# arkworks-rs/circom-compat

Hardware: NVIDIA H100
Metric: groth16_proofs_per_sec_bn254_2p20 (higher is better)
Workload: dtype u32x8 (254-bit Montgomery integers)

## Files before the change

### circom_compat_b200/csrc/msm.cu

```cuda
#include <algorithm>
#include <type_traits>
#include <vector>
#include "msm.cuh"
#include "util.cuh"

namespace b2g {

std::atomic<uint64_t> g_launch_count{0};

template <class C, class F>
__global__ void __launch_bounds__(128) msm_table_kernel(const void* __restrict__ bases, uint32_t n, int c, int nwin, void* __restrict__ table) {
    uint32_t i = blockIdx.x * blockDim.x + threadIdx.x;
    if (i >= n) return;
    using Pt = typename C::Pt; using Aff = typename C::Aff; using E = typename F::elem;
    Aff p = aff_load<F>(bases, i);
    if (C::aff_is_inf(p)) {
        Aff z; z.x = F::zero(); z.y = F::zero();
        for (int w = 0; w < nwin; w++) aff_store<F>(table, (size_t)w * n + i, z);
        return;
    }
    Pt pts[MSM_MAX_WIN];
    E pre[MSM_MAX_WIN];
    Pt cur = C::from_affine(p);
    E acc = F::one();
    for (int w = 0; w < nwin; w++) {
        pts[w] = cur;
        pre[w] = acc;
        acc = F::mul(acc, cur.zzz);
        if (w + 1 < nwin) for (int j = 0; j < c; j++) cur = C::dbl(cur);
    }
    E inv = F::inv(acc);
    for (int w = nwin - 1; w >= 0; w--) {
        E iz = F::mul(inv, pre[w]);
        inv = F::mul(inv, pts[w].zzz);
        Aff a;
        a.y = F::mul(pts[w].y, iz);
        a.x = F::mul(pts[w].x, F::mul(F::sqr(pts[w].zz), F::sqr(iz)));
        aff_store<F>(table, (size_t)w * n + i, a);
    }
}

template <class C, class F>
__global__ void __launch_bounds__(256) msm_validate_kernel(const void* __restrict__ bases, uint32_t n, uint32_t* __restrict__ bad) {
    uint32_t i = blockIdx.x * blockDim.x + threadIdx.x;
    if (i >= n) return;
    if (!aff_on_curve<C, F>(aff_load<F>(bases, i))) atomicMax(bad, i + 1u);
}

__global__ void __launch_bounds__(256) msm_canon_kernel(const fe* __restrict__ scalars, uint32_t n, uint32_t scalar_stride, int scalars_mont, fe* __restrict__ canon_out) {
    uint32_t i = blockIdx.x * blockDim.x + threadIdx.x;
    if (i >= n) return;
    scalars += (size_t)blockIdx.y * scalar_stride;
    canon_out += (size_t)blockIdx.y * n;
    fe k = fe_load_nc(&scalars[i]);
    if (scalars_mont) k = Fr::to_canonical(k);
    fe_store(&canon_out[i], k);
}

__device__ __forceinline__ uint32_t msm_window_bits(const uint32_t* __restrict__ k, int c, int w) {
    const uint32_t off = (uint32_t)w * (uint32_t)c, limb = off >> 5, sh = off & 31u;
    if (limb >= 8) return 0u;
    uint64_t v = __ldg(&k[limb]);
    if (limb + 1 < 8 && sh + (uint32_t)c > 32u) v |= (uint64_t)__ldg(&k[limb + 1]) << 32;
    return (uint32_t)(v >> sh) & ((1u << c) - 1u);
}

__device__ __forceinline__ int32_t msm_digit_at(const uint32_t* __restrict__ k, int c, int w) {
    const uint32_t half = 1u << (c - 1);
    uint32_t carry = 0;
    for (int v = w - 1; v >= 0; v--) {
        const uint32_t b = msm_window_bits(k, c, v);
        if (b >= half) { carry = 1; break; }
        if (b < half - 1) break;
    }
    const uint32_t coef = msm_window_bits(k, c, w) + carry;
    const uint32_t cout = (coef + half) >> c;
    return (int32_t)coef - (int32_t)(cout << c);
}

constexpr int MSM_LEADER_ROUNDS = 2;

__global__ void __launch_bounds__(256) msm_count_kernel(const fe* __restrict__ canon, uint32_t n, int c, int nwin, uint32_t nb, uint32_t* __restrict__ counts) {
    canon += (size_t)blockIdx.y * n;
    counts += (size_t)blockIdx.y * nb;
    const uint64_t tid = (uint64_t)blockIdx.x * blockDim.x + threadIdx.x;
    const uint32_t w = (uint32_t)(tid / n), i = (uint32_t)(tid % n);
    int32_t d = 0;
    if (w < (uint32_t)nwin) d = msm_digit_at(canon[i].l, c, (int)w);
    const uint32_t b = d ? (uint32_t)(d < 0 ? -d : d) - 1u : 0xffffffffu;
    const uint32_t lane = threadIdx.x & 31;
    bool pending = d != 0;
    {
        const uint32_t hot = __ballot_sync(0xffffffffu, pending && b == 0u);
        if (hot) {
            if ((int)lane == __ffs(hot) - 1) atomicAdd(&counts[0], (uint32_t)__popc(hot));
            if (b == 0u) pending = false;
        }
    }
    #pragma unroll
    for (int round = 0; round < MSM_LEADER_ROUNDS; round++) {
        const uint32_t pend = __ballot_sync(0xffffffffu, pending);
        if (!pend) break;
        const int leader = __ffs(pend) - 1;
        const uint32_t lb = __shfl_sync(0xffffffffu, b, leader);
        const bool mine = pending && b == lb;
        const uint32_t same = __ballot_sync(0xffffffffu, mine);
        if ((int)lane == leader) atomicAdd(&counts[lb], (uint32_t)__popc(same));
        if (mine) pending = false;
    }
    if (pending) atomicAdd(&counts[b], 1u);
}

__global__ void __launch_bounds__(1024) msm_scan_kernel(const uint32_t* __restrict__ counts, uint32_t nb, uint32_t* __restrict__ offsets,
                                                        uint32_t* __restrict__ cursor) {
    __shared__ uint32_t warp_sums[32];
    __shared__ uint32_t carry_s;
    const uint32_t tid = threadIdx.x, per = (nb + 1023u) / 1024u;
    const uint32_t lo = tid * per, hi = min(lo + per, nb);
    uint32_t s = 0;
    if ((per & 3u) == 0 && hi == lo + per) {
        const uint4* v4 = reinterpret_cast<const uint4*>(counts + lo);
        #pragma unroll 4
        for (uint32_t j = 0; j < per / 4; j++) { const uint4 q = __ldg(&v4[j]); s += q.x + q.y + q.z + q.w; }
    } else {
        for (uint32_t j = lo; j < hi; j++) s += counts[j];
    }
    uint32_t v = s;
    #pragma unroll
    for (int d = 1; d < 32; d <<= 1) { uint32_t t = __shfl_up_sync(0xffffffffu, v, d); if ((tid & 31) >= (uint32_t)d) v += t; }
    if ((tid & 31) == 31) warp_sums[tid >> 5] = v;
    __syncthreads();
    if (tid < 32) {
        uint32_t w = warp_sums[tid], x = w;
        #pragma unroll
        for (int d = 1; d < 32; d <<= 1) { uint32_t t = __shfl_up_sync(0xffffffffu, x, d); if (tid >= (uint32_t)d) x += t; }
        warp_sums[tid] = x - w;
        if (tid == 31) carry_s = x;
    }
    __syncthreads();
    uint32_t run = warp_sums[tid >> 5] + v - s;
    for (uint32_t j = lo; j < hi; j++) { offsets[j] = run; cursor[j] = 0; run += counts[j]; }
    if (tid == 0) offsets[nb] = carry_s;
}

__global__ void __launch_bounds__(256) msm_scatter_kernel(const fe* __restrict__ canon, uint32_t n, uint32_t row_stride, int c, int nwin, uint32_t nb,
                                   const uint32_t* __restrict__ offsets, uint32_t* __restrict__ cursor, uint32_t* __restrict__ entries) {
    canon += (size_t)blockIdx.y * n;
    offsets += (size_t)blockIdx.y * nb;
    cursor += (size_t)blockIdx.y * nb;
    const uint64_t tid = (uint64_t)blockIdx.x * blockDim.x + threadIdx.x;
    const uint32_t w = (uint32_t)(tid / n), i = (uint32_t)(tid % n);
    int32_t d = 0;
    if (w < (uint32_t)nwin) d = msm_digit_at(canon[i].l, c, (int)w);
    const uint32_t b = d ? (uint32_t)(d < 0 ? -d : d) - 1u : 0xffffffffu;
    const uint32_t lane = threadIdx.x & 31;
    const uint32_t entry = (w * row_stride + i) | (d < 0 ? 0x80000000u : 0u);
    bool pending = d != 0;
    {
        const uint32_t hot = __ballot_sync(0xffffffffu, pending && b == 0u);
        if (hot) {
            const int leader = __ffs(hot) - 1;
            uint32_t base = 0;
            if ((int)lane == leader) base = atomicAdd(&cursor[0], (uint32_t)__popc(hot));
            base = __shfl_sync(0xffffffffu, base, leader);
            if (pending && b == 0u) {
                entries[offsets[0] + base + (uint32_t)__popc(hot & ((1u << lane) - 1u))] = entry;
                pending = false;
            }
        }
    }
    #pragma unroll
    for (int round = 0; round < MSM_LEADER_ROUNDS; round++) {
        const uint32_t pend = __ballot_sync(0xffffffffu, pending);
        if (!pend) break;
        const int leader = __ffs(pend) - 1;
        const uint32_t lb = __shfl_sync(0xffffffffu, b, leader);
        const bool mine = pending && b == lb;
        const uint32_t same = __ballot_sync(0xffffffffu, mine);
        uint32_t base = 0;
        if ((int)lane == leader) base = atomicAdd(&cursor[lb], (uint32_t)__popc(same));
        base = __shfl_sync(0xffffffffu, base, leader);
        if (mine) {
            entries[offsets[b] + base + (uint32_t)__popc(same & ((1u << lane) - 1u))] = entry;
            pending = false;
        }
    }
    if (pending) entries[offsets[b] + atomicAdd(&cursor[b], 1u)] = entry;
}

__global__ void __launch_bounds__(1024) msm_aff_levels_kernel(uint32_t nb, int rounds, uint32_t* const* __restrict__ off) {
    __shared__ uint32_t warp_sums[32];
    __shared__ uint32_t carry_s;
    const uint32_t tid = threadIdx.x, per = (nb + 1023u) / 1024u;
    const uint32_t lo = min(tid * per, nb), hi = min(lo + per, nb);
    for (int k = 1; k <= rounds; k++) {
        const uint32_t* prev = off[k - 1];
        uint32_t* cur = off[k];
        uint32_t s = 0;
        for (uint32_t j = lo; j < hi; j++) s += (prev[j + 1] - prev[j] + 1u) >> 1;
        uint32_t v = s;
        #pragma unroll
        for (int d = 1; d < 32; d <<= 1) { uint32_t t = __shfl_up_sync(0xffffffffu, v, d); if ((tid & 31) >= (uint32_t)d) v += t; }
        if ((tid & 31) == 31) warp_sums[tid >> 5] = v;
        __syncthreads();
        if (tid < 32) {
            uint32_t w = warp_sums[tid], x = w;
            #pragma unroll
            for (int d = 1; d < 32; d <<= 1) { uint32_t t = __shfl_up_sync(0xffffffffu, x, d); if (tid >= (uint32_t)d) x += t; }
            warp_sums[tid] = x - w;
            if (tid == 31) carry_s = x;
        }
        __syncthreads();
        uint32_t run = warp_sums[tid >> 5] + v - s;
        for (uint32_t j = lo; j < hi; j++) { cur[j] = run; run += (prev[j + 1] - prev[j] + 1u) >> 1; }
        if (tid == 0) cur[nb] = carry_s;
        __syncthreads();
    }
}

__global__ void __launch_bounds__(256) msm_aff_src_kernel(const uint32_t* __restrict__ off_prev, const uint32_t* __restrict__ off_cur, uint32_t nb,
                                                          uint32_t* __restrict__ src) {
    const uint32_t total = off_cur[nb];
    for (uint32_t q = blockIdx.x * blockDim.x + threadIdx.x; q < total; q += gridDim.x * blockDim.x) {
        uint32_t lo = 0, hi = nb;
        while (hi - lo > 1) { const uint32_t mid = (lo + hi) >> 1; if (off_cur[mid] <= q) lo = mid; else hi = mid; }
        const uint32_t j = q - off_cur[lo];
        const uint32_t p0 = off_prev[lo], cnt = off_prev[lo + 1] - p0;
        src[q] = (p0 + 2u * j) | ((2u * j + 1u < cnt) ? 0x80000000u : 0u);
    }
}

enum : int { AFF_COPY_P = 0, AFF_COPY_Q = 1, AFF_INF = 2, AFF_ADD = 3, AFF_DBL = 4 };

template <class C, class F, bool LEVEL0>
__device__ __forceinline__ int aff_fetch(const void* __restrict__ table, const uint32_t* __restrict__ entries, const void* __restrict__ prev,
                                         uint32_t s, typename C::Aff& P, typename C::Aff& Q, typename F::elem& d) {
    const uint32_t i0 = s & 0x7fffffffu;
    const bool pair = (s >> 31) != 0;
    if (LEVEL0) {
        const uint32_t e0 = entries[i0];
        P = aff_load<F>(table, (size_t)(e0 & 0x7fffffffu));
        if (e0 >> 31) P.y = F::neg(P.y);
        if (pair) {
            const uint32_t e1 = entries[i0 + 1];
            Q = aff_load<F>(table, (size_t)(e1 & 0x7fffffffu));
            if (e1 >> 31) Q.y = F::neg(Q.y);
        }
    } else {
        P = aff_load<F>(prev, (size_t)i0);
        if (pair) Q = aff_load<F>(prev, (size_t)i0 + 1);
    }
    if (!pair) return AFF_COPY_P;
    if (C::aff_is_inf(P)) return AFF_COPY_Q;
    if (C::aff_is_inf(Q)) return AFF_COPY_P;
    if (F::eq(P.x, Q.x)) {
        if (F::eq(P.y, Q.y) && !F::is_zero(P.y)) { d = F::dbl(P.y); return AFF_DBL; }
        return AFF_INF;
    }
    d = F::sub(Q.x, P.x);
    return AFF_ADD;
}

template <class C, class F, bool LEVEL0>
__global__ void __launch_bounds__(128) msm_aff_prod_kernel(const void* __restrict__ table, const uint32_t* __restrict__ entries, const void* __restrict__ prev,
                                                           const uint32_t* __restrict__ src, const uint32_t* __restrict__ off_cur, uint32_t nb,
                                                           void* __restrict__ pref, void* __restrict__ totals) {
    using E = typename F::elem; using Aff = typename C::Aff;
    const uint32_t total = off_cur[nb];
    const uint32_t t = blockIdx.x * blockDim.x + threadIdx.x, stride = gridDim.x * blockDim.x;
    E run = F::one();
// ... 298 lines not shown
            for (int i = top; i >= 0; i--) { m = C::dbl(m); if ((base >> i) & 1u) C::add(m, run); }
            C::add(acc, m);
        }
    }
    Pt r = block_sum_points<C, F, TailThreads<F>::N>(acc, sh);
    if (threadIdx.x == 0) pt_store<F>(partials, blockIdx.x, r);
}

template <class C, class F>
__global__ void __launch_bounds__(TailThreads<F>::N) msm_sum_kernel(const void* __restrict__ pts, uint32_t count, void* __restrict__ out, size_t out_stride) {
    using Pt = typename C::Pt;
    extern __shared__ __align__(32) unsigned char smem_raw[];
    Pt* sh = reinterpret_cast<Pt*>(smem_raw);
    pts = (const char*)pts + (size_t)blockIdx.x * count * sizeof(Pt);
    out = (char*)out + (size_t)blockIdx.x * out_stride;
    Pt acc = C::infinity();
    for (uint32_t i = threadIdx.x; i < count; i += TailThreads<F>::N) { Pt q = pt_load<F>(pts, i); C::add(acc, q); }
    Pt r = block_sum_points<C, F, TailThreads<F>::N>(acc, sh);
    if (threadIdx.x == 0) pt_store<F>(out, 0, r);
}

static uint32_t env_u32(const char* name, uint32_t dflt) {
    const char* v = getenv(name);
    if (!v || !*v) return dflt;
    long x = strtol(v, nullptr, 10);
    return x > 0 ? (uint32_t)x : dflt;
}

void msm_validate_points(const void* pts_dev, uint32_t n, bool g2, cudaStream_t st, const char* what) {
    if (n == 0) return;
    struct Flag { uint32_t* d = nullptr; ~Flag() { if (d) cudaFree(d); } } flag;
    uint32_t bad = 0;
    CUDA_CHECK(cudaMalloc(&flag.d, 4));
    CUDA_CHECK(cudaMemsetAsync(flag.d, 0, 4, st));
    if (g2) msm_validate_kernel<G2, Fq2><<<(n + 255) / 256, 256, 0, st>>>(pts_dev, n, flag.d);
    else msm_validate_kernel<G1, Fq><<<(n + 255) / 256, 256, 0, st>>>(pts_dev, n, flag.d);
    g_launch_count += 1;
    CUDA_CHECK(cudaMemcpyAsync(&bad, flag.d, 4, cudaMemcpyDeviceToHost, st));
    CUDA_CHECK(cudaStreamSynchronize(st));
    if (bad) throw_error(B2G_E_INPUT, std::string(g2 ? "G2" : "G1") + " point " + std::to_string(bad - 1) + " of " + what + " is not on the curve");
}

template <class C, class F>
static void msm_build_table_t(MsmPlan& plan, const void* bases_dev, uint32_t n, cudaStream_t st) {
    const size_t aff = 2 * Bytes<F>::ELEM;
    uint32_t c = env_u32("B2G_MSM_C", (uint32_t)msm_pick_c(n ? n : 1));
    if (c < 8 || c > 22) throw_error(B2G_E_SHAPE, "B2G_MSM_C must be in [8, 22]");
    plan.n = n; plan.c = (int)c; plan.nwin = msm_nwin(plan.c); plan.nbuckets = 1u << (plan.c - 1);
    if (n == 0) { plan.table = nullptr; return; }
    if ((uint64_t)n * plan.nwin >= (1ull << 31)) throw_error(B2G_E_SHAPE, "msm: n * windows exceeds 2^31 table rows");
    msm_validate_points(bases_dev, n, plan.g2, st, "the query slice");
    CUDA_CHECK(cudaMalloc(&plan.table, (size_t)n * plan.nwin * aff));
    msm_table_kernel<C, F><<<(n + 127) / 128, 128, 0, st>>>(bases_dev, n, plan.c, plan.nwin, plan.table);
    g_launch_count += 1;
    CUDA_CHECK(cudaGetLastError());
}

void msm_build_table(MsmPlan& plan, const void* bases_dev, uint32_t n, bool g2, cudaStream_t st) {
    plan.g2 = g2;
    if (g2) msm_build_table_t<G2, Fq2>(plan, bases_dev, n, st);
    else msm_build_table_t<G1, Fq>(plan, bases_dev, n, st);
}

void msm_free_table(MsmPlan& plan) { if (plan.table) cudaFree(plan.table); plan.table = nullptr; }

void msm_scratch_alloc(MsmScratch& s, uint32_t n, int nwin, uint32_t nbuckets_one, bool g2, bool with_sort, uint32_t count) {
    s.g2 = g2; s.cap_n = n; s.cap_nwin = nwin; s.cap_buckets = nbuckets_one; s.cap_count = count;
    s.chunk = env_u32(g2 ? "B2G_MSM_CHUNK_G2" : "B2G_MSM_CHUNK", env_u32("B2G_MSM_CHUNK", 64));
    const size_t pt = (g2 ? 4 * 64 : 4 * 32);
    const size_t nent = (size_t)n * nwin * count;
    const size_t nbuckets = (size_t)nbuckets_one * count;
    const size_t nchunks = (nent + s.chunk - 1) / s.chunk + 1;
    s.reduce_chunk = env_u32("B2G_MSM_REDUCE_CHUNK", MSM_REDUCE_CHUNK_DEFAULT);
    {
        const char* bulk_env = getenv("B2G_ACC_BULK");
        s.bulk = bulk_env && *bulk_env ? *bulk_env == '1' : !g2;
    }
    const size_t npart = ((size_t)nbuckets_one / (s.reduce_chunk * 32) + 64) * count;
    if (with_sort) {
        CUDA_CHECK(cudaMalloc(&s.counts, (size_t)nbuckets * 4));
        CUDA_CHECK(cudaMalloc(&s.offsets, ((size_t)nbuckets + 1) * 4));
        CUDA_CHECK(cudaMalloc(&s.cursor, (size_t)nbuckets * 4));
        CUDA_CHECK(cudaMalloc(&s.entries, (nent + 8) * 4));
        CUDA_CHECK(cudaMalloc(&s.scalars_canon, ((size_t)n * count + 1) * sizeof(fe)));
    }
    CUDA_CHECK(cudaMalloc(&s.big_list, (size_t)nbuckets * 4));
    CUDA_CHECK(cudaMalloc(&s.big_count, 4));
    CUDA_CHECK(cudaMalloc(&s.frag_first, nchunks * pt));
    CUDA_CHECK(cudaMalloc(&s.frag_last, nchunks * pt));
    CUDA_CHECK(cudaMalloc(&s.buckets, (size_t)nbuckets * pt));
    CUDA_CHECK(cudaMalloc(&s.partials, (npart + 1) * pt));
    CUDA_CHECK(cudaMalloc(&s.result, pt)); s.result_owned = true;
    {
        int rounds = 0;
        const char* ov = getenv("B2G_MSM_AFFINE_ROUNDS");
        if (ov && *ov) { long x = strtol(ov, nullptr, 10); rounds = x < 0 ? 0 : (x > MSM_AFF_MAX_ROUNDS ? MSM_AFF_MAX_ROUNDS : (int)x); }
        s.aff_cap_rounds = rounds;
        s.aff_nmax[0] = (uint32_t)nent;
        for (int k = 1; k <= rounds; k++) s.aff_nmax[k] = s.aff_nmax[k - 1] / 2 + (uint32_t)(nbuckets / 2) + 1;
        if (rounds) {
            const size_t elem = g2 ? 64 : 32, aff = 2 * elem;
            if (with_sort) {
                std::vector<uint32_t*> offs(MSM_AFF_MAX_ROUNDS + 1, nullptr);
                offs[0] = s.offsets;
                for (int k = 1; k <= rounds; k++) {
                    CUDA_CHECK(cudaMalloc(&s.aff_off[k], ((size_t)nbuckets + 1) * 4));
                    CUDA_CHECK(cudaMalloc(&s.aff_src[k], ((size_t)s.aff_nmax[k] + 1) * 4));
                    offs[k] = s.aff_off[k];
                }
                s.aff_off[0] = s.offsets;
                CUDA_CHECK(cudaMalloc(&s.aff_off_dev, (MSM_AFF_MAX_ROUNDS + 1) * sizeof(uint32_t*)));
                CUDA_CHECK(cudaMemcpy(s.aff_off_dev, offs.data(), (MSM_AFF_MAX_ROUNDS + 1) * sizeof(uint32_t*), cudaMemcpyHostToDevice));
            }
            CUDA_CHECK(cudaMalloc(&s.aff_list[0], ((size_t)s.aff_nmax[1] + 1) * aff));
            if (rounds > 1) CUDA_CHECK(cudaMalloc(&s.aff_list[1], ((size_t)s.aff_nmax[2] + 1) * aff));
            const size_t threads1 = ((size_t)s.aff_nmax[1] + MSM_AFF_M - 1) / MSM_AFF_M + 128;
            CUDA_CHECK(cudaMalloc(&s.aff_pref, ((size_t)s.aff_nmax[1] + 1) * elem));
            CUDA_CHECK(cudaMalloc(&s.aff_totals, threads1 * elem));
            CUDA_CHECK(cudaMalloc(&s.aff_tscratch, threads1 * elem));
        }
    }
    if (env_u32("B2G_MSM_TAIL_PRIORITY", 1) == 1) {
        int least = 0, greatest = 0;
        CUDA_CHECK(cudaDeviceGetStreamPriorityRange(&least, &greatest));
        CUDA_CHECK(cudaStreamCreateWithPriority(&s.tail, cudaStreamNonBlocking, greatest));
        CUDA_CHECK(cudaEventCreateWithFlags(&s.ev_acc, cudaEventDisableTiming));
        CUDA_CHECK(cudaEventCreateWithFlags(&s.ev_tail, cudaEventDisableTiming));
    }
}

void msm_scratch_free(MsmScratch& s) {
    void* ptrs[] = {s.counts, s.offsets, s.cursor, s.entries, s.big_list, s.big_count, s.frag_first, s.frag_last,
                    s.buckets, s.partials, s.result_owned ? s.result : nullptr, s.scalars_canon,
                    s.aff_list[0], s.aff_list[1], s.aff_pref, s.aff_totals, s.aff_tscratch, s.aff_off_dev};
    for (void* p : ptrs) if (p) cudaFree(p);
    for (int k = 1; k <= MSM_AFF_MAX_ROUNDS; k++) { if (s.aff_off[k]) cudaFree(s.aff_off[k]); if (s.aff_src[k]) cudaFree(s.aff_src[k]); }
    if (s.tail) { cudaStreamDestroy(s.tail); cudaEventDestroy(s.ev_acc); cudaEventDestroy(s.ev_tail); }
    s = MsmScratch();
}

void msm_sort(const MsmPlan& plan, MsmScratch& s, const fe* scalars_dev, uint32_t n, bool scalars_mont, cudaStream_t st, uint32_t count,
              uint32_t scalar_stride) {
    if (n > plan.n) n = plan.n;
    s.sorted_n = n; s.sorted_count = count;
    if (n == 0 || plan.table == nullptr) return;
    if (n > s.cap_n || plan.nwin > s.cap_nwin || plan.nbuckets > s.cap_buckets || count > s.cap_count || !s.entries) throw_error(B2G_E_SHAPE, "msm: sort scratch too small");
    const uint32_t nb = plan.nbuckets * count;
    constexpr unsigned SORT_CTA = 256;
    CUDA_CHECK(cudaMemsetAsync(s.counts, 0, (size_t)nb * 4, st));
    const dim3 pair_grid((unsigned)(((uint64_t)n * plan.nwin + SORT_CTA - 1) / SORT_CTA), count);
    msm_canon_kernel<<<dim3((n + SORT_CTA - 1) / SORT_CTA, count), SORT_CTA, 0, st>>>(scalars_dev, n, scalar_stride ? scalar_stride : n, scalars_mont ? 1 : 0, s.scalars_canon);
    msm_count_kernel<<<pair_grid, SORT_CTA, 0, st>>>(s.scalars_canon, n, plan.c, plan.nwin, plan.nbuckets, s.counts);
    msm_scan_kernel<<<1, 1024, 0, st>>>(s.counts, nb, s.offsets, s.cursor);
    msm_scatter_kernel<<<pair_grid, SORT_CTA, 0, st>>>(s.scalars_canon, n, plan.n, plan.c, plan.nwin, plan.nbuckets, s.offsets, s.cursor, s.entries);
    g_launch_count += 4;
    s.aff_rounds = s.aff_off_dev ? s.aff_cap_rounds : 0;
    if (s.aff_rounds) {
        msm_aff_levels_kernel<<<1, 1024, 0, st>>>(nb, s.aff_rounds, s.aff_off_dev);
        for (int k = 1; k <= s.aff_rounds; k++) {
            const unsigned blocks = (unsigned)std::min<uint64_t>(((uint64_t)s.aff_nmax[k] + 255) / 256, 1u << 20);
            msm_aff_src_kernel<<<blocks, 256, 0, st>>>(s.aff_off[k - 1], s.aff_off[k], nb, s.aff_src[k]);
        }
        g_launch_count += 1 + s.aff_rounds;
    }
    CUDA_CHECK(cudaGetLastError());
}

template <class C, class F>
static void launch_accumulate(const void* table, const uint32_t* entries, const uint32_t* offsets, uint32_t nb, uint32_t chunk, uint32_t nruns,
                              const MsmScratch& s, bool bulk, cudaStream_t st) {
    constexpr bool g2 = std::is_same<F, Fq2>::value;
    constexpr uint32_t runs_per_cta = g2 ? 64u : 128u;
    const uint32_t slab_words = bulk && (size_t)chunk * runs_per_cta * 4 <= MSM_SLAB_MAX_BYTES ? chunk * runs_per_cta : 0u;
    const unsigned blocks = (unsigned)(((uint64_t)nruns + runs_per_cta - 1) / runs_per_cta);
    if constexpr (g2)
        msm_accumulate_g2_kernel<<<blocks, 128, (size_t)slab_words * 4, st>>>(table, entries, offsets, nb, chunk, s.buckets, s.frag_first, s.frag_last, slab_words);
    else
        msm_accumulate_kernel<C, F><<<blocks, 128, (size_t)slab_words * 4, st>>>(table, entries, offsets, nb, chunk, s.buckets, s.frag_first, s.frag_last, slab_words);
}

template <class C, class F>
static void msm_accumulate_t(const MsmPlan& plan, const MsmScratch& sorted, MsmScratch& s, cudaStream_t st) {
    using Pt = typename C::Pt;
    const size_t ptb = sizeof(Pt);
    const uint32_t n = sorted.sorted_n, count = sorted.sorted_count;
    const size_t rstride = s.result_stride ? s.result_stride : ptb;
    if (n == 0 || plan.table == nullptr) { CUDA_CHECK(cudaMemset2DAsync(s.result, rstride, 0, ptb, count, st)); return; }
    if (plan.nbuckets > s.cap_buckets || n > s.cap_n || plan.nwin > s.cap_nwin || count > s.cap_count) throw_error(B2G_E_SHAPE, "msm: accumulate scratch too small");
    const uint32_t nb = plan.nbuckets * count, chunk = s.chunk;
    CUDA_CHECK(cudaMemsetAsync(s.big_count, 0, 4, st));
    const uint64_t nent = (uint64_t)n * plan.nwin * count;
    const uint32_t nthreads = (uint32_t)((nent + chunk - 1) / chunk);
    if (s.prof0) CUDA_CHECK(cudaEventRecord(s.prof0, st));
    int rounds = sorted.aff_rounds < s.aff_cap_rounds ? sorted.aff_rounds : s.aff_cap_rounds;
    if (rounds && (sorted.aff_nmax[1] > s.aff_nmax[1] || !s.aff_list[0])) rounds = 0;
    const uint32_t* offsets = sorted.offsets;
    if (rounds) {
        const void* prev = nullptr;
        for (int k = 1; k <= rounds; k++) {
            const uint32_t nk = sorted.aff_nmax[k];
            const unsigned blocks = (unsigned)(((uint64_t)nk + (uint64_t)MSM_AFF_M * 128 - 1) / ((uint64_t)MSM_AFF_M * 128));
            const uint32_t stride = blocks * 128u, U = (stride + MSM_AFF_S - 1) / MSM_AFF_S;
            void* out = s.aff_list[(k - 1) & 1];
            if (k == 1) {
                msm_aff_prod_kernel<C, F, true><<<blocks, 128, 0, st>>>(plan.table, sorted.entries, nullptr, sorted.aff_src[k], sorted.aff_off[k], nb, s.aff_pref, s.aff_totals);
                msm_aff_invert_kernel<F><<<(U + 63) / 64, 64, 0, st>>>(s.aff_totals, s.aff_tscratch, stride, U);
                msm_aff_apply_kernel<C, F, true><<<blocks, 128, 0, st>>>(plan.table, sorted.entries, nullptr, sorted.aff_src[k], sorted.aff_off[k], nb, s.aff_pref, s.aff_totals, out);
            } else {
                msm_aff_prod_kernel<C, F, false><<<blocks, 128, 0, st>>>(nullptr, nullptr, prev, sorted.aff_src[k], sorted.aff_off[k], nb, s.aff_pref, s.aff_totals);
                msm_aff_invert_kernel<F><<<(U + 63) / 64, 64, 0, st>>>(s.aff_totals, s.aff_tscratch, stride, U);
                msm_aff_apply_kernel<C, F, false><<<blocks, 128, 0, st>>>(nullptr, nullptr, prev, sorted.aff_src[k], sorted.aff_off[k], nb, s.aff_pref, s.aff_totals, out);
            }
            prev = out;
        }
        g_launch_count += 3 * rounds;
        offsets = sorted.aff_off[rounds];
        const uint32_t nthreads_r = (uint32_t)(((uint64_t)sorted.aff_nmax[rounds] + chunk - 1) / chunk);
        launch_accumulate<C, F>(prev, nullptr, offsets, nb, chunk, nthreads_r, s, false, st);
    } else {
        launch_accumulate<C, F>(plan.table, sorted.entries, sorted.offsets, nb, chunk, nthreads, s, s.bulk, st);
    }
    if (s.prof1) CUDA_CHECK(cudaEventRecord(s.prof1, st));
    cudaStream_t main_st = st;
    if (s.tail) { CUDA_CHECK(cudaEventRecord(s.ev_acc, st)); CUDA_CHECK(cudaStreamWaitEvent(s.tail, s.ev_acc, 0)); st = s.tail; }
    msm_fold_kernel<C, F><<<(nb + 127) / 128, 128, 0, st>>>(offsets, nb, chunk, s.buckets, s.frag_first, s.frag_last, s.big_list, s.big_count);
    constexpr int NT = TailThreads<F>::N;
    const size_t sh = (size_t)NT * ptb;
    msm_fold_big_kernel<C, F><<<128, NT, sh, st>>>(offsets, chunk, s.buckets, s.frag_first, s.frag_last, s.big_list, s.big_count);
    const uint32_t rchunk = s.reduce_chunk, nb1 = plan.nbuckets;
    const uint32_t nred = (nb1 + rchunk - 1) / rchunk;
    const uint32_t npart = (nred + NT - 1) / NT;
    msm_reduce_kernel<C, F><<<dim3(npart, count), NT, sh, st>>>(s.buckets, nb1, rchunk, s.partials);
    msm_sum_kernel<C, F><<<count, NT, sh, st>>>(s.partials, npart, s.result, rstride);
    if (s.tail) { CUDA_CHECK(cudaEventRecord(s.ev_tail, s.tail)); CUDA_CHECK(cudaStreamWaitEvent(main_st, s.ev_tail, 0)); }
    g_launch_count += 5;
    CUDA_CHECK(cudaGetLastError());
}

// ... 18 lines not shown
```

### circom_compat_b200/csrc/msm.cuh

```cuda
#pragma once
#include "ec.cuh"

namespace b2g {

constexpr int MSM_MAX_WIN = 32;
constexpr int MSM_BIG_FRAGS = 32;

struct MsmPlan {
    uint32_t n = 0;
    int c = 0, nwin = 0;
    uint32_t nbuckets = 0;
    void* table = nullptr;
    bool g2 = false;
};

constexpr int MSM_AFF_MAX_ROUNDS = 6;
constexpr int MSM_AFF_M = 16;
constexpr int MSM_AFF_S = 64;

struct MsmScratch {
    uint32_t cap_n = 0; int cap_nwin = 0; uint32_t cap_buckets = 0; uint32_t chunk = 64; uint32_t sorted_n = 0; uint32_t reduce_chunk = 8;
    uint32_t cap_count = 1, sorted_count = 1;
    size_t result_stride = 0;
    uint32_t *counts = nullptr, *offsets = nullptr, *cursor = nullptr, *entries = nullptr;
    uint32_t *big_list = nullptr, *big_count = nullptr;
    void *frag_first = nullptr, *frag_last = nullptr, *buckets = nullptr, *partials = nullptr, *result = nullptr;
    fe* scalars_canon = nullptr;
    bool g2 = false, result_owned = false;
    bool bulk = false;
    cudaEvent_t prof0 = nullptr, prof1 = nullptr;
    cudaStream_t tail = nullptr;
    cudaEvent_t ev_acc = nullptr, ev_tail = nullptr;
    int aff_rounds = 0;
    int aff_cap_rounds = 0;
    uint32_t aff_nmax[MSM_AFF_MAX_ROUNDS + 1] = {};
    uint32_t* aff_off[MSM_AFF_MAX_ROUNDS + 1] = {};
    uint32_t** aff_off_dev = nullptr;
    uint32_t* aff_src[MSM_AFF_MAX_ROUNDS + 1] = {};
    void* aff_list[2] = {nullptr, nullptr};
    void *aff_pref = nullptr, *aff_totals = nullptr, *aff_tscratch = nullptr;
};

inline int msm_pick_c(uint32_t n) {
    if (n >= 3u << 18) return 17;
    if (n >= 1u << 19) return 16;
    if (n >= 1u << 15) return 15;
    if (n >= 1u << 13) return 13;
    if (n >= 1u << 11) return 11;
    int lg = 0; while ((1ull << (lg + 1)) <= n) lg++;
    return lg - 3 < 8 ? 8 : lg - 3;
}
inline int msm_nwin(int c) { return (255 + c - 1) / c; }

}
```

### circom_compat_b200/csrc/prover.cu

```cuda
#include <atomic>
#include <chrono>
#include <cstring>
#include <vector>
#include "../../include/b2groth.h"
#include "ec.cuh"
#include "msm.cuh"
#include "fixed.cuh"
#include "ntt.cuh"
#include "util.cuh"
#include "verify.cuh"

namespace b2g {

void msm_build_table(MsmPlan& plan, const void* bases_dev, uint32_t n, bool g2, cudaStream_t st);
void msm_free_table(MsmPlan& plan);
void msm_scratch_alloc(MsmScratch& s, uint32_t n, int nwin, uint32_t nbuckets, bool g2, bool with_sort, uint32_t count = 1);
void msm_sort(const MsmPlan& plan, MsmScratch& s, const fe* scalars_dev, uint32_t n, bool scalars_mont, cudaStream_t st, uint32_t count = 1,
              uint32_t scalar_stride = 0);
void msm_accumulate(const MsmPlan& plan, const MsmScratch& sorted, MsmScratch& acc, cudaStream_t st);
void msm_scratch_free(MsmScratch& s);
void msm_run(const MsmPlan& plan, MsmScratch& s, const fe* scalars_dev, uint32_t n, bool scalars_mont, cudaStream_t st, uint32_t count = 1,
             uint32_t scalar_stride = 0);
void msm_init_kernels();
void msm_validate_points(const void* pts_dev, uint32_t n, bool g2, cudaStream_t st, const char* what);
// ... 32 lines not shown
    uint64_t alloc_gen = 1;
    uint64_t g_launches[2] = {0, 0};
    unsigned long long* d_epoch = nullptr;
    uint8_t* d_xchg = nullptr;
    size_t eval_cap = 0, eval_common = 0;
    uint8_t** d_peer_ptrs = nullptr;
    void* peer_mapped[64] = {};
    int peers_imported = 0;
    VerifyBufs* vbufs = nullptr;
};

static std::atomic<uint64_t> g_next_uid{1};

struct b2g_pk {
    uint64_t uid = g_next_uid++;
    int device = 0, shard_rank = 0, shard_count = 1;
    uint32_t n_vars = 0, n_public = 0, domain = 0;
    MsmPlan plan[NQ];
    uint32_t lo[NQ] = {}, cnt[NQ] = {}, scalar_off[NQ] = {};
    uint8_t* d_consts = nullptr;
    void *d_tab_delta1 = nullptr, *d_tab_delta2 = nullptr;
    void *d_tab_aa = nullptr, *d_tab_bb = nullptr;
    uint32_t* d_bidx = nullptr;
    uint32_t b_compact = 0;
};

struct b2g_mat {
    uint64_t uid = g_next_uid++;
    int device = 0;
    uint32_t m = 0, num_inputs = 0, n_vars = 0, n = 0;
    int logn = 0;
    NttDomain dom;
    uint32_t *a_rowptr = nullptr, *a_col = nullptr, *b_rowptr = nullptr, *b_col = nullptr, *c_rowptr = nullptr, *c_col = nullptr;
    fe *a_val = nullptr, *b_val = nullptr, *c_val = nullptr;
    uint32_t reduction = B2G_REDUCTION_CIRCOM;
};

namespace b2g {

thread_local std::string g_last_error;

struct Scalar256 { uint32_t l[8]; };

CtxView ctx_view(b2g_ctx* ctx) { return {ctx->device, ctx->st[0], ctx->pending_out != nullptr, &ctx->vbufs}; }

constexpr size_t PRE_BYTES = 4 * 128 + 256;
__global__ void __launch_bounds__(192) glue_pre_kernel(const void* __restrict__ tab_d1, const void* __restrict__ tab_d2, const void* __restrict__ tab_aa,
                                                       const void* __restrict__ tab_bb, const Scalar256* __restrict__ rs, uint8_t* __restrict__ pre) {
    __shared__ G1::Pt sh1[5][32];
    __shared__ G2::Pt sh2[32];
    __shared__ G1::Pt res[5];
    rs += 2 * blockIdx.x;
    pre += (size_t)blockIdx.x * PRE_BYTES;
    const Scalar256 r = rs[0], s = rs[1];
    const int warp = threadIdx.x >> 5;
    const bool lead = (threadIdx.x & 31) == 0;
    if (warp < 5) {
        Scalar256 k = (warp == 0 || warp == 4) ? r : s;
        if (warp == 2) {
            fe rc, sc;
            #pragma unroll
            for (int i = 0; i < 8; i++) { rc.l[i] = r.l[i]; sc.l[i] = s.l[i]; }
            fe rm = Fr::from_canonical(rc), sm = Fr::from_canonical(sc);
            fe rs_ = Fr::to_canonical(Fr::mul(rm, sm));
            #pragma unroll
            for (int i = 0; i < 8; i++) k.l[i] = rs_.l[i];
        }
        const void* tab = warp < 3 ? tab_d1 : (warp == 3 ? tab_aa : tab_bb);
        G1::Pt p = warp_fixed_mul<G1, Fq>(tab, k.l, sh1[warp]);
        if (lead) { res[warp] = p; if (warp < 3) pt_store<Fq>(pre, warp, p); }
    } else {
        G2::Pt p = warp_fixed_mul<G2, Fq2>(tab_d2, s.l, sh2);
        if (lead) pt_store<Fq2>(pre + 4 * 128, 0, p);
    }
    __syncthreads();
    if (threadIdx.x == 0) {
        G1::Pt kc = res[2];
        G1::add(kc, res[3]);
        G1::add(kc, res[4]);
        pt_store<Fq>(pre, 3, kc);
    }
}

__global__ void scale_partial_kernel(const uint8_t* __restrict__ pt, const Scalar256* __restrict__ k, uint8_t* __restrict__ out) {
    if (threadIdx.x != 0) return;
    pt += blockIdx.x * REC_BYTES; out += blockIdx.x * REC_BYTES; k += 2 * blockIdx.x;
    const Scalar256 kk = *k;
    G1::Pt p = pt_load<Fq>(pt, 0);
    pt_store<Fq>(out, 0, G1::mul_scalar(p, kk.l));
}

__device__ __forceinline__ void store_canon(uint8_t* out, int slot, const fe& v) { fe_store(out + 32 * slot, Fq::to_canonical(v)); }

__global__ void glue_post_kernel(const uint8_t* __restrict__ partials, int count, int stride, int scaled_off, const uint8_t* __restrict__ consts,
                                 const uint8_t* __restrict__ pre, const Scalar256* __restrict__ rs, uint8_t* __restrict__ proof) {
    __shared__ G1::Pt shA, shB1, shsA, shrB1;
    partials += (size_t)blockIdx.x * count * stride;
    pre += (size_t)blockIdx.x * PRE_BYTES;
    rs += 2 * blockIdx.x;
    proof += (size_t)blockIdx.x * 256;
    const Scalar256 r = rs[0], s = rs[1];
    const int warp = threadIdx.x >> 5;
    const bool lead = (threadIdx.x & 31) == 0;
    const bool legacy = scaled_off < 0;
    if (lead && (warp == 0 || (warp == 1 && legacy))) {
        G1::Pt acc = pt_load<Fq>(pre, warp);
        G1::madd(acc, aff_load<Fq>(consts, warp == 0 ? 3 : 4));
        for (int k = 0; k < count; k++) { G1::Pt q = pt_load<Fq>(partials + (size_t)k * stride + (warp == 0 ? 256 : 384), 0); G1::add(acc, q); }
        G1::madd(acc, aff_load<Fq>(consts, warp == 0 ? 0 : 1));
        if (warp == 0) shA = acc; else shB1 = acc;
        if (warp == 0 && !legacy) {
            G1::Aff a = G1::to_affine(acc);
            store_canon(proof, 0, a.x); store_canon(proof, 1, a.y);
        }
    }
    if (lead && warp == 1 && !legacy) {
        G1::Pt acc = pt_load<Fq>(pre, 3);
        for (int k = 0; k < count; k++) {
            const uint8_t* rec = partials + (size_t)k * stride;
            G1::Pt q = pt_load<Fq>(rec + scaled_off, 0); G1::add(acc, q);
            q = pt_load<Fq>(rec + scaled_off + 128, 0); G1::add(acc, q);
            q = pt_load<Fq>(rec + 128, 0); G1::add(acc, q);
            q = pt_load<Fq>(rec, 0); G1::add(acc, q);
        }
        G1::Aff c = G1::to_affine(acc);
        store_canon(proof, 6, c.x); store_canon(proof, 7, c.y);
    }
    if (lead && warp == 2) {
        G2::Pt acc = pt_load<Fq2>(pre + 4 * 128, 0);
        G2::madd(acc, aff_load<Fq2>(consts + 5 * 64, 2));
        for (int k = 0; k < count; k++) { G2::Pt q = pt_load<Fq2>(partials + (size_t)k * stride + 512, 0); G2::add(acc, q); }
        G2::madd(acc, aff_load<Fq2>(consts + 5 * 64, 0));
        G2::Aff b = G2::to_affine(acc);
        store_canon(proof, 2, b.x.c0); store_canon(proof, 3, b.x.c1); store_canon(proof, 4, b.y.c0); store_canon(proof, 5, b.y.c1);
    }
    if (!legacy) return;
    __syncthreads();
    if (lead && warp == 0) shsA = G1::mul_scalar(shA, s.l);
    if (lead && warp == 1) shrB1 = G1::mul_scalar(shB1, r.l);
    if (lead && warp == 3) {
        G1::Aff a = G1::to_affine(shA);
        store_canon(proof, 0, a.x); store_canon(proof, 1, a.y);
    }
    __syncthreads();
    if (lead && warp == 0) {
        G1::Pt acc = shsA;
        G1::add(acc, shrB1);
        G1::Pt rsd = G1::neg(pt_load<Fq>(pre, 2));
        G1::add(acc, rsd);
        for (int k = 0; k < count; k++) {
            G1::Pt l = pt_load<Fq>(partials + (size_t)k * stride + 128, 0); G1::add(acc, l);
            G1::Pt h = pt_load<Fq>(partials + (size_t)k * stride, 0); G1::add(acc, h);
        }
        G1::Aff c = G1::to_affine(acc);
        store_canon(proof, 6, c.x); store_canon(proof, 7, c.y);
    }
}

constexpr size_t XCHG_SLOT = 256 + REC_BYTES;
constexpr size_t XCHG_BYTES = 2 * XCHG_SLOT;
constexpr size_t EVAL_FLAG_OFF = XCHG_BYTES + 64;
constexpr size_t EVAL_OFF = XCHG_BYTES + 256;
constexpr int MAP_RANKS = 3;

__device__ __forceinline__ unsigned long long ld_acquire_sys(const unsigned long long* p) {
    unsigned long long v;
    asm volatile("ld.acquire.sys.global.u64 %0, [%1];" : "=l"(v) : "l"(p) : "memory");
    return v;
}
__device__ __forceinline__ void st_release_sys(unsigned long long* p, unsigned long long v) {
    asm volatile("st.release.sys.global.u64 [%0], %1;" :: "l"(p), "l"(v) : "memory");
}
// ... 1202 lines not shown
```

Baseline: 42.27.

## Fuse scalar canonicalization into MSM sort, tile the bucket scan, parallelize partial scaling

Count and scatter kernels now run one thread per scalar and walk all windows with a carried signed-digit state. This removes the separate canonicalization kernel, its buffer, and the per-window carry recomputation, at the cost of less parallelism per thread and a serial window loop. The single-block bucket scan becomes a two-kernel tiled multi-block scan. The scale_partial kernel replaces its single-thread double-and-add with one lane building a doubling ladder in shared memory, then 32 lanes summing the set bits and tree-reducing.

```diff
diff --git a/circom_compat_b200/csrc/msm.cu b/circom_compat_b200/csrc/msm.cu
--- a/circom_compat_b200/csrc/msm.cu
+++ b/circom_compat_b200/csrc/msm.cu
@@ -47,145 +47,194 @@
     if (!aff_on_curve<C, F>(aff_load<F>(bases, i))) atomicMax(bad, i + 1u);
 }
 
-__global__ void __launch_bounds__(256) msm_canon_kernel(const fe* __restrict__ scalars, uint32_t n, uint32_t scalar_stride, int scalars_mont, fe* __restrict__ canon_out) {
-    uint32_t i = blockIdx.x * blockDim.x + threadIdx.x;
-    if (i >= n) return;
+struct MsmDigitWalk {
+    uint32_t k[8];
+    uint32_t carry = 0;
+    int c;
+
+    __device__ __forceinline__ MsmDigitWalk(const fe* __restrict__ scalars, uint32_t i, bool valid, bool mont, int c_) : c(c_) {
+        fe v = fe_zero();
+        if (valid) { v = fe_load_nc(&scalars[i]); if (mont) v = Fr::to_canonical(v); }
+        #pragma unroll
+        for (int j = 0; j < 8; j++) k[j] = v.l[j];
+    }
+
+    __device__ __forceinline__ uint32_t bits(int w) const {
+        const uint32_t off = (uint32_t)w * (uint32_t)c, limb = off >> 5, sh = off & 31u;
+        uint32_t lo = 0, hi = 0;
+        #pragma unroll
+        for (int j = 0; j < 8; j++) { if ((uint32_t)j == limb) lo = k[j]; if ((uint32_t)j == limb + 1) hi = k[j]; }
+        const uint64_t v = ((uint64_t)hi << 32) | lo;
+        return (uint32_t)(v >> sh) & ((1u << c) - 1u);
+    }
+
+    __device__ __forceinline__ int32_t next(int w) {
+        const uint32_t half = 1u << (c - 1);
+        const uint32_t coef = bits(w) + carry;
+        carry = (coef + half) >> c;
+        return (int32_t)coef - (int32_t)(carry << c);
+    }
+};
+
+__device__ __forceinline__ uint32_t msm_digit_bucket(int32_t d) { return d ? (uint32_t)(d < 0 ? -d : d) - 1u : 0xffffffffu; }
+
+constexpr int MSM_LEADER_ROUNDS = 2;
+
+__global__ void __launch_bounds__(256) msm_count_kernel(const fe* __restrict__ scalars, uint32_t n, uint32_t scalar_stride, int scalars_mont,
+                                                        int c, int nwin, uint32_t nb, uint32_t* __restrict__ counts) {
     scalars += (size_t)blockIdx.y * scalar_stride;
-    canon_out += (size_t)blockIdx.y * n;
-    fe k = fe_load_nc(&scalars[i]);
-    if (scalars_mont) k = Fr::to_canonical(k);
-    fe_store(&canon_out[i], k);
-}
-
-__device__ __forceinline__ uint32_t msm_window_bits(const uint32_t* __restrict__ k, int c, int w) {
-    const uint32_t off = (uint32_t)w * (uint32_t)c, limb = off >> 5, sh = off & 31u;
-    if (limb >= 8) return 0u;
-    uint64_t v = __ldg(&k[limb]);
-    if (limb + 1 < 8 && sh + (uint32_t)c > 32u) v |= (uint64_t)__ldg(&k[limb + 1]) << 32;
-    return (uint32_t)(v >> sh) & ((1u << c) - 1u);
-}
-
-__device__ __forceinline__ int32_t msm_digit_at(const uint32_t* __restrict__ k, int c, int w) {
-    const uint32_t half = 1u << (c - 1);
-    uint32_t carry = 0;
-    for (int v = w - 1; v >= 0; v--) {
-        const uint32_t b = msm_window_bits(k, c, v);
-        if (b >= half) { carry = 1; break; }
-        if (b < half - 1) break;
-    }
-    const uint32_t coef = msm_window_bits(k, c, w) + carry;
-    const uint32_t cout = (coef + half) >> c;
-    return (int32_t)coef - (int32_t)(cout << c);
-}
-
-constexpr int MSM_LEADER_ROUNDS = 2;
-
-__global__ void __launch_bounds__(256) msm_count_kernel(const fe* __restrict__ canon, uint32_t n, int c, int nwin, uint32_t nb, uint32_t* __restrict__ counts) {
-    canon += (size_t)blockIdx.y * n;
     counts += (size_t)blockIdx.y * nb;
-    const uint64_t tid = (uint64_t)blockIdx.x * blockDim.x + threadIdx.x;
-    const uint32_t w = (uint32_t)(tid / n), i = (uint32_t)(tid % n);
-    int32_t d = 0;
-    if (w < (uint32_t)nwin) d = msm_digit_at(canon[i].l, c, (int)w);
-    const uint32_t b = d ? (uint32_t)(d < 0 ? -d : d) - 1u : 0xffffffffu;
+    const uint32_t i = blockIdx.x * blockDim.x + threadIdx.x;
+    MsmDigitWalk walk(scalars, i, i < n, scalars_mont != 0, c);
     const uint32_t lane = threadIdx.x & 31;
-    bool pending = d != 0;
-    {
-        const uint32_t hot = __ballot_sync(0xffffffffu, pending && b == 0u);
-        if (hot) {
-            if ((int)lane == __ffs(hot) - 1) atomicAdd(&counts[0], (uint32_t)__popc(hot));
-            if (b == 0u) pending = false;
-        }
-    }
+    #pragma unroll 1
+    for (int w = 0; w < nwin; w++) {
+        const int32_t d = walk.next(w);
+        const uint32_t b = msm_digit_bucket(d);
+        bool pending = d != 0;
+        {
+            const uint32_t hot = __ballot_sync(0xffffffffu, pending && b == 0u);
+            if (hot) {
+                if ((int)lane == __ffs(hot) - 1) atomicAdd(&counts[0], (uint32_t)__popc(hot));
+                if (b == 0u) pending = false;
+            }
+        }
+        #pragma unroll
+        for (int round = 0; round < MSM_LEADER_ROUNDS; round++) {
+            const uint32_t pend = __ballot_sync(0xffffffffu, pending);
+            if (!pend) break;
+            const int leader = __ffs(pend) - 1;
+            const uint32_t lb = __shfl_sync(0xffffffffu, b, leader);
+            const bool mine = pending && b == lb;
+            const uint32_t same = __ballot_sync(0xffffffffu, mine);
+            if ((int)lane == leader) atomicAdd(&counts[lb], (uint32_t)__popc(same));
+            if (mine) pending = false;
+        }
+        if (pending) atomicAdd(&counts[b], 1u);
+    }
+}
+
+constexpr uint32_t MSM_SCAN_THREADS = 1024;
+constexpr uint32_t MSM_SCAN_PER = 4;
+constexpr uint32_t MSM_SCAN_TILE = MSM_SCAN_THREADS * MSM_SCAN_PER;
+
+__device__ __forceinline__ uint32_t scan_load4(const uint32_t* __restrict__ counts, uint32_t nb, uint32_t lo, uint32_t q[MSM_SCAN_PER]) {
+    if (lo + MSM_SCAN_PER <= nb && (lo & 3u) == 0) {
+        const uint4 v = __ldg(reinterpret_cast<const uint4*>(counts + lo));
+        q[0] = v.x; q[1] = v.y; q[2] = v.z; q[3] = v.w;
+    } else {
+        #pragma unroll
+        for (uint32_t j = 0; j < MSM_SCAN_PER; j++) q[j] = lo + j < nb ? counts[lo + j] : 0u;
+    }
+    return q[0] + q[1] + q[2] + q[3];
+}
+
+__device__ __forceinline__ uint32_t scan_block_sum(uint32_t v, uint32_t* red) {
     #pragma unroll
-    for (int round = 0; round < MSM_LEADER_ROUNDS; round++) {
-        const uint32_t pend = __ballot_sync(0xffffffffu, pending);
-        if (!pend) break;
-        const int leader = __ffs(pend) - 1;
-        const uint32_t lb = __shfl_sync(0xffffffffu, b, leader);
-        const bool mine = pending && b == lb;
-        const uint32_t same = __ballot_sync(0xffffffffu, mine);
-        if ((int)lane == leader) atomicAdd(&counts[lb], (uint32_t)__popc(same));
-        if (mine) pending = false;
-    }
-    if (pending) atomicAdd(&counts[b], 1u);
-}
-
-__global__ void __launch_bounds__(1024) msm_scan_kernel(const uint32_t* __restrict__ counts, uint32_t nb, uint32_t* __restrict__ offsets,
-                                                        uint32_t* __restrict__ cursor) {
-    __shared__ uint32_t warp_sums[32];
-    __shared__ uint32_t carry_s;
-    const uint32_t tid = threadIdx.x, per = (nb + 1023u) / 1024u;
-    const uint32_t lo = tid * per, hi = min(lo + per, nb);
-    uint32_t s = 0;
-    if ((per & 3u) == 0 && hi == lo + per) {
-        const uint4* v4 = reinterpret_cast<const uint4*>(counts + lo);
-        #pragma unroll 4
-        for (uint32_t j = 0; j < per / 4; j++) { const uint4 q = __ldg(&v4[j]); s += q.x + q.y + q.z + q.w; }
-    } else {
-        for (uint32_t j = lo; j < hi; j++) s += counts[j];
-    }
-    uint32_t v = s;
+    for (int d = 16; d > 0; d >>= 1) v += __shfl_xor_sync(0xffffffffu, v, d);
+    if ((threadIdx.x & 31) == 0) red[threadIdx.x >> 5] = v;
+    __syncthreads();
+    uint32_t t = red[threadIdx.x & 31];
     #pragma unroll
-    for (int d = 1; d < 32; d <<= 1) { uint32_t t = __shfl_up_sync(0xffffffffu, v, d); if ((tid & 31) >= (uint32_t)d) v += t; }
-    if ((tid & 31) == 31) warp_sums[tid >> 5] = v;
+    for (int d = 16; d > 0; d >>= 1) t += __shfl_xor_sync(0xffffffffu, t, d);
     __syncthreads();
-    if (tid < 32) {
-        uint32_t w = warp_sums[tid], x = w;
-        #pragma unroll
-        for (int d = 1; d < 32; d <<= 1) { uint32_t t = __shfl_up_sync(0xffffffffu, x, d); if (tid >= (uint32_t)d) x += t; }
-        warp_sums[tid] = x - w;
-        if (tid == 31) carry_s = x;
-    }
+    return t;
+}
+
+__device__ __forceinline__ uint32_t scan_block_exclusive(uint32_t v, uint32_t* red) {
+    const uint32_t lane = threadIdx.x & 31;
+    uint32_t x = v;
+    #pragma unroll
+    for (int d = 1; d < 32; d <<= 1) { const uint32_t t = __shfl_up_sync(0xffffffffu, x, d); if (lane >= (uint32_t)d) x += t; }
+    if (lane == 31) red[threadIdx.x >> 5] = x;
     __syncthreads();
-    uint32_t run = warp_sums[tid >> 5] + v - s;
-    for (uint32_t j = lo; j < hi; j++) { offsets[j] = run; cursor[j] = 0; run += counts[j]; }
-    if (tid == 0) offsets[nb] = carry_s;
-}
-
-__global__ void __launch_bounds__(256) msm_scatter_kernel(const fe* __restrict__ canon, uint32_t n, uint32_t row_stride, int c, int nwin, uint32_t nb,
+    const uint32_t w = red[lane];
+    uint32_t y = w;
+    #pragma unroll
+    for (int d = 1; d < 32; d <<= 1) { const uint32_t t = __shfl_up_sync(0xffffffffu, y, d); if (lane >= (uint32_t)d) y += t; }
+    const uint32_t warp_before = __shfl_sync(0xffffffffu, y - w, threadIdx.x >> 5);
+    __syncthreads();
+    return warp_before + x - v;
+}
+
+__global__ void __launch_bounds__(MSM_SCAN_THREADS) msm_scan_tiles_kernel(const uint32_t* __restrict__ counts, uint32_t nb, uint32_t* __restrict__ tile_sums) {
+    __shared__ uint32_t red[32];
+    uint32_t q[MSM_SCAN_PER];
+    const uint32_t s = scan_block_sum(scan_load4(counts, nb, blockIdx.x * MSM_SCAN_TILE + threadIdx.x * MSM_SCAN_PER, q), red);
+    if (threadIdx.x == 0) tile_sums[blockIdx.x] = s;
+}
+
+__global__ void __launch_bounds__(MSM_SCAN_THREADS) msm_scan_offsets_kernel(const uint32_t* __restrict__ counts, uint32_t nb, const uint32_t* __restrict__ tile_sums,
+                                                                          uint32_t* __restrict__ offsets, uint32_t* __restrict__ cursor) {
+    __shared__ uint32_t red[32];
+    uint32_t c = 0;
+    for (uint32_t t = threadIdx.x; t < blockIdx.x; t += MSM_SCAN_THREADS) c += tile_sums[t];
+    const uint32_t carry_in = scan_block_sum(c, red);
+    const uint32_t lo = blockIdx.x * MSM_SCAN_TILE + threadIdx.x * MSM_SCAN_PER;
+    uint32_t q[MSM_SCAN_PER];
+    const uint32_t s = scan_load4(counts, nb, lo, q);
+    uint32_t run = carry_in + scan_block_exclusive(s, red);
+    #pragma unroll
+    for (uint32_t j = 0; j < MSM_SCAN_PER; j++) {
+        if (lo + j < nb) { offsets[lo + j] = run; cursor[lo + j] = 0; }
+        run += q[j];
+    }
+    if (blockIdx.x == gridDim.x - 1 && threadIdx.x == MSM_SCAN_THREADS - 1) offsets[nb] = run;
+}
+
+static void msm_scan(const uint32_t* counts, uint32_t nb, uint32_t* offsets, uint32_t* cursor, uint32_t* tile_sums, cudaStream_t st) {
+    const unsigned tiles = (unsigned)((nb + MSM_SCAN_TILE - 1) / MSM_SCAN_TILE);
+    msm_scan_tiles_kernel<<<tiles, MSM_SCAN_THREADS, 0, st>>>(counts, nb, tile_sums);
+    msm_scan_offsets_kernel<<<tiles, MSM_SCAN_THREADS, 0, st>>>(counts, nb, tile_sums, offsets, cursor);
+    g_launch_count += 2;
+}
+
+__global__ void __launch_bounds__(256) msm_scatter_kernel(const fe* __restrict__ scalars, uint32_t n, uint32_t scalar_stride, int scalars_mont,
+                                   uint32_t row_stride, int c, int nwin, uint32_t nb,
                                    const uint32_t* __restrict__ offsets, uint32_t* __restrict__ cursor, uint32_t* __restrict__ entries) {
-    canon += (size_t)blockIdx.y * n;
+    scalars += (size_t)blockIdx.y * scalar_stride;
     offsets += (size_t)blockIdx.y * nb;
     cursor += (size_t)blockIdx.y * nb;
-    const uint64_t tid = (uint64_t)blockIdx.x * blockDim.x + threadIdx.x;
-    const uint32_t w = (uint32_t)(tid / n), i = (uint32_t)(tid % n);
-    int32_t d = 0;
-    if (w < (uint32_t)nwin) d = msm_digit_at(canon[i].l, c, (int)w);
-    const uint32_t b = d ? (uint32_t)(d < 0 ? -d : d) - 1u : 0xffffffffu;
+    const uint32_t i = blockIdx.x * blockDim.x + threadIdx.x;
+    MsmDigitWalk walk(scalars, i, i < n, scalars_mont != 0, c);
     const uint32_t lane = threadIdx.x & 31;
-    const uint32_t entry = (w * row_stride + i) | (d < 0 ? 0x80000000u : 0u);
-    bool pending = d != 0;
-    {
-        const uint32_t hot = __ballot_sync(0xffffffffu, pending && b == 0u);
-        if (hot) {
-            const int leader = __ffs(hot) - 1;
+    #pragma unroll 1
+    for (int w = 0; w < nwin; w++) {
+        const int32_t d = walk.next(w);
+        const uint32_t b = msm_digit_bucket(d);
+        const uint32_t entry = ((uint32_t)w * row_stride + i) | (d < 0 ? 0x80000000u : 0u);
+        bool pending = d != 0;
+        {
+            const uint32_t hot = __ballot_sync(0xffffffffu, pending && b == 0u);
+            if (hot) {
+                const int leader = __ffs(hot) - 1;
+                uint32_t base = 0;
+                if ((int)lane == leader) base = atomicAdd(&cursor[0], (uint32_t)__popc(hot));
+                base = __shfl_sync(0xffffffffu, base, leader);
+                if (pending && b == 0u) {
+                    entries[offsets[0] + base + (uint32_t)__popc(hot & ((1u << lane) - 1u))] = entry;
+                    pending = false;
+                }
+            }
+        }
+        #pragma unroll
+        for (int round = 0; round < MSM_LEADER_ROUNDS; round++) {
+            const uint32_t pend = __ballot_sync(0xffffffffu, pending);
+            if (!pend) break;
+            const int leader = __ffs(pend) - 1;
+            const uint32_t lb = __shfl_sync(0xffffffffu, b, leader);
+            const bool mine = pending && b == lb;
+            const uint32_t same = __ballot_sync(0xffffffffu, mine);
             uint32_t base = 0;
-            if ((int)lane == leader) base = atomicAdd(&cursor[0], (uint32_t)__popc(hot));
+            if ((int)lane == leader) base = atomicAdd(&cursor[lb], (uint32_t)__popc(same));
             base = __shfl_sync(0xffffffffu, base, leader);
-            if (pending && b == 0u) {
-                entries[offsets[0] + base + (uint32_t)__popc(hot & ((1u << lane) - 1u))] = entry;
+            if (mine) {
+                entries[offsets[b] + base + (uint32_t)__popc(same & ((1u << lane) - 1u))] = entry;
                 pending = false;
             }
         }
-    }
-    #pragma unroll
-    for (int round = 0; round < MSM_LEADER_ROUNDS; round++) {
-        const uint32_t pend = __ballot_sync(0xffffffffu, pending);
-        if (!pend) break;
-        const int leader = __ffs(pend) - 1;
-        const uint32_t lb = __shfl_sync(0xffffffffu, b, leader);
-        const bool mine = pending && b == lb;
-        const uint32_t same = __ballot_sync(0xffffffffu, mine);
-        uint32_t base = 0;
-        if ((int)lane == leader) base = atomicAdd(&cursor[lb], (uint32_t)__popc(same));
-        base = __shfl_sync(0xffffffffu, base, leader);
-        if (mine) {
-            entries[offsets[b] + base + (uint32_t)__popc(same & ((1u << lane) - 1u))] = entry;
-            pending = false;
-        }
-    }
-    if (pending) entries[offsets[b] + atomicAdd(&cursor[b], 1u)] = entry;
+        if (pending) entries[offsets[b] + atomicAdd(&cursor[b], 1u)] = entry;
+    }
 }
 
 __global__ void __launch_bounds__(1024) msm_aff_levels_kernel(uint32_t nb, int rounds, uint32_t* const* __restrict__ off) {
@@ -650,7 +699,7 @@
         CUDA_CHECK(cudaMalloc(&s.offsets, ((size_t)nbuckets + 1) * 4));
         CUDA_CHECK(cudaMalloc(&s.cursor, (size_t)nbuckets * 4));
         CUDA_CHECK(cudaMalloc(&s.entries, (nent + 8) * 4));
-        CUDA_CHECK(cudaMalloc(&s.scalars_canon, ((size_t)n * count + 1) * sizeof(fe)));
+        CUDA_CHECK(cudaMalloc(&s.scan_tiles, ((size_t)nbuckets + MSM_SCAN_TILE - 1) / MSM_SCAN_TILE * 4));
     }
     CUDA_CHECK(cudaMalloc(&s.big_list, (size_t)nbuckets * 4));
     CUDA_CHECK(cudaMalloc(&s.big_count, 4));
@@ -699,7 +748,7 @@
 
 void msm_scratch_free(MsmScratch& s) {
     void* ptrs[] = {s.counts, s.offsets, s.cursor, s.entries, s.big_list, s.big_count, s.frag_first, s.frag_last,
-                    s.buckets, s.partials, s.result_owned ? s.result : nullptr, s.scalars_canon,
+                    s.buckets, s.partials, s.result_owned ? s.result : nullptr, s.scan_tiles,
                     s.aff_list[0], s.aff_list[1], s.aff_pref, s.aff_totals, s.aff_tscratch, s.aff_off_dev};
     for (void* p : ptrs) if (p) cudaFree(p);
     for (int k = 1; k <= MSM_AFF_MAX_ROUNDS; k++) { if (s.aff_off[k]) cudaFree(s.aff_off[k]); if (s.aff_src[k]) cudaFree(s.aff_src[k]); }
@@ -716,12 +765,12 @@
     const uint32_t nb = plan.nbuckets * count;
     constexpr unsigned SORT_CTA = 256;
     CUDA_CHECK(cudaMemsetAsync(s.counts, 0, (size_t)nb * 4, st));
-    const dim3 pair_grid((unsigned)(((uint64_t)n * plan.nwin + SORT_CTA - 1) / SORT_CTA), count);
-    msm_canon_kernel<<<dim3((n + SORT_CTA - 1) / SORT_CTA, count), SORT_CTA, 0, st>>>(scalars_dev, n, scalar_stride ? scalar_stride : n, scalars_mont ? 1 : 0, s.scalars_canon);
-    msm_count_kernel<<<pair_grid, SORT_CTA, 0, st>>>(s.scalars_canon, n, plan.c, plan.nwin, plan.nbuckets, s.counts);
-    msm_scan_kernel<<<1, 1024, 0, st>>>(s.counts, nb, s.offsets, s.cursor);
-    msm_scatter_kernel<<<pair_grid, SORT_CTA, 0, st>>>(s.scalars_canon, n, plan.n, plan.c, plan.nwin, plan.nbuckets, s.offsets, s.cursor, s.entries);
-    g_launch_count += 4;
+    const dim3 grid((n + SORT_CTA - 1) / SORT_CTA, count);
+    const uint32_t stride = scalar_stride ? scalar_stride : n;
+    msm_count_kernel<<<grid, SORT_CTA, 0, st>>>(scalars_dev, n, stride, scalars_mont ? 1 : 0, plan.c, plan.nwin, plan.nbuckets, s.counts);
+    msm_scan(s.counts, nb, s.offsets, s.cursor, s.scan_tiles, st);
+    msm_scatter_kernel<<<grid, SORT_CTA, 0, st>>>(scalars_dev, n, stride, scalars_mont ? 1 : 0, plan.n, plan.c, plan.nwin, plan.nbuckets, s.offsets, s.cursor, s.entries);
+    g_launch_count += 2;
     s.aff_rounds = s.aff_off_dev ? s.aff_cap_rounds : 0;
     if (s.aff_rounds) {
         msm_aff_levels_kernel<<<1, 1024, 0, st>>>(nb, s.aff_rounds, s.aff_off_dev);
diff --git a/circom_compat_b200/csrc/msm.cuh b/circom_compat_b200/csrc/msm.cuh
--- a/circom_compat_b200/csrc/msm.cuh
+++ b/circom_compat_b200/csrc/msm.cuh
@@ -25,7 +25,7 @@
     uint32_t *counts = nullptr, *offsets = nullptr, *cursor = nullptr, *entries = nullptr;
     uint32_t *big_list = nullptr, *big_count = nullptr;
     void *frag_first = nullptr, *frag_last = nullptr, *buckets = nullptr, *partials = nullptr, *result = nullptr;
-    fe* scalars_canon = nullptr;
+    uint32_t* scan_tiles = nullptr;
     bool g2 = false, result_owned = false;
     bool bulk = false;
     cudaEvent_t prof0 = nullptr, prof1 = nullptr;
diff --git a/circom_compat_b200/csrc/prover.cu b/circom_compat_b200/csrc/prover.cu
--- a/circom_compat_b200/csrc/prover.cu
+++ b/circom_compat_b200/csrc/prover.cu
@@ -138,12 +138,32 @@
     }
 }
 
-__global__ void scale_partial_kernel(const uint8_t* __restrict__ pt, const Scalar256* __restrict__ k, uint8_t* __restrict__ out) {
-    if (threadIdx.x != 0) return;
+__global__ void __launch_bounds__(32) scale_partial_kernel(const uint8_t* __restrict__ pt, const Scalar256* __restrict__ k, uint8_t* __restrict__ out) {
+    __shared__ G1::Pt ladder[256];
+    __shared__ G1::Pt sh[32];
     pt += blockIdx.x * REC_BYTES; out += blockIdx.x * REC_BYTES; k += 2 * blockIdx.x;
+    const uint32_t lane = threadIdx.x & 31;
     const Scalar256 kk = *k;
-    G1::Pt p = pt_load<Fq>(pt, 0);
-    pt_store<Fq>(out, 0, G1::mul_scalar(p, kk.l));
+    int top = 255;
+    while (top >= 0 && !((kk.l[top >> 5] >> (top & 31)) & 1u)) top--;
+    if (lane == 0) {
+        G1::Pt p = pt_load<Fq>(pt, 0);
+        #pragma unroll 1
+        for (int i = 0; i <= top; i++) { ladder[i] = p; if (i < top) p = G1::dbl(p); }
+    }
+    __syncwarp();
+    G1::Pt acc = G1::infinity();
+    #pragma unroll 1
+    for (int i = (int)lane; i <= top; i += 32)
+        if ((kk.l[i >> 5] >> (i & 31)) & 1u) { const G1::Pt q = ladder[i]; G1::add(acc, q); }
+    sh[lane] = acc;
+    __syncwarp();
+    #pragma unroll 1
+    for (int d = 16; d > 0; d >>= 1) {
+        if ((int)lane < d) { G1::Pt a = sh[lane]; const G1::Pt q = sh[lane + d]; G1::add(a, q); sh[lane] = a; }
+        __syncwarp();
+    }
+    if (lane == 0) pt_store<Fq>(out, 0, sh[0]);
 }
 
 __device__ __forceinline__ void store_canon(uint8_t* out, int slot, const fe& v) { fe_store(out + 32 * slot, Fq::to_canonical(v)); }
```

New measurement: 43.34, median of 6. 2.5% higher.
